# weiaicunzai/pytorch-camvid

Measured on AMD Instinct MI355X. Metric: images/sec fwd+bwd UNet 3x360x480 bs=8, higher is better.
Workload: dtype f32; 1 GPU; UNET(3,12) train fwd+bwd+CE, per-GPU batch 8 x 3x360x480 fp32 (BASELINE.json configs[1]); global_batch=8, parallelism=dp1

## Files before the change

pytorch-camvid_amd/csrc/pointwise.hip:

```cpp
#include "cvk_common.h"

namespace {

inline int grid_for(long total) {
    const long b = (total + 255) / 256;
    return (int)(b < 16384 ? (b > 0 ? b : 1) : 16384);
}

#define CVK_GRID_STRIDE(i, total) \
    for (long i = (long)blockIdx.x * blockDim.x + threadIdx.x; i < (total); i += (long)gridDim.x * blockDim.x)

__global__ void k_import_small(const float* __restrict__ src, int64_t sN, int64_t sC, int64_t sH, int64_t sW,
                               float* __restrict__ dst, int N, int C, int H, int W) {
    const long total = (long)N * H * W;
    CVK_GRID_STRIDE(i, total) {
        const int x = (int)(i % W);
        const long t = i / W;
        const int y = (int)(t % H), n = (int)(t / H);
        const float* p = src + n * sN + y * sH + x * sW;
        f32x4 v = {0.f, 0.f, 0.f, 0.f};
        for (int c = 0; c < C; ++c) v[c] = p[c * sC];
        *reinterpret_cast<f32x4*>(dst + i * 4) = v;
    }
}
// ... 279 lines not shown
        const int yo = (int)(t % Ho);
        t /= Ho;
        const int c = (int)(t % C), n = (int)(t / C);
        const int k = code[(((long)n * Ho + yo) * Wo + xo) * C + c];
        idx[i] = (int64_t)(2 * yo + (k >> 1)) * W + 2 * xo + (k & 1);
    }
}

struct Tap { int i0, i1; float l0, l1; };
__device__ __forceinline__ Tap make_tap(int dst, float scale, int n_in) {
    Tap t;
    const float src = scale * (float)dst;
    t.i0 = (int)src;
    if (t.i0 > n_in - 1) t.i0 = n_in - 1;
    t.i1 = t.i0 + (t.i0 < n_in - 1 ? 1 : 0);
    t.l1 = src - (float)t.i0;
    t.l0 = 1.f - t.l1;
    return t;
}

struct RowDiv {
    unsigned lo, hi_mask;
    explicit RowDiv(unsigned d) {
        const unsigned long long m = 0x100000000ULL / d + 1ULL;
        lo = (unsigned)m;
        hi_mask = (m >> 32) ? 0xFFFFFFFFu : 0u;
    }
    __device__ __forceinline__ unsigned div(unsigned t) const { return __umulhi(t, lo) + (t & hi_mask); }
};

template <int V>
__global__ __launch_bounds__(256) void k_bilinear_fwd(const float* __restrict__ x, float* __restrict__ out, int H, int W, int C,
                                                     float sy, float sx, RowDiv dcv) {
    typedef typename VT_<V>::T VT;
    const int Wo = 2 * W, cvn = C / V;
    const int yo = blockIdx.y, n = blockIdx.z;
    const unsigned idx = blockIdx.x * 256 + threadIdx.x;
    if (idx >= (unsigned)(Wo * cvn)) return;
    const int xo = (int)dcv.div(idx), cv = (int)idx - xo * cvn;
    const Tap ty = make_tap(yo, sy, H), tx = make_tap(xo, sx, W);
    const float* b = x + ((long)n * H * W) * C + cv * V;
    VT v00 = *reinterpret_cast<const VT*>(b + ((long)ty.i0 * W + tx.i0) * C);
    VT v01 = *reinterpret_cast<const VT*>(b + ((long)ty.i0 * W + tx.i1) * C);
    VT v10 = *reinterpret_cast<const VT*>(b + ((long)ty.i1 * W + tx.i0) * C);
    VT v11 = *reinterpret_cast<const VT*>(b + ((long)ty.i1 * W + tx.i1) * C);
    VT o;
#pragma unroll
    for (int j = 0; j < V; ++j)
        el<V>(o, j) = ty.l0 * (tx.l0 * el<V>(v00, j) + tx.l1 * el<V>(v01, j)) +
                      ty.l1 * (tx.l0 * el<V>(v10, j) + tx.l1 * el<V>(v11, j));
    *reinterpret_cast<VT*>(out + (((long)n * 2 * H + yo) * Wo) * C + (long)idx * V) = o;
}

constexpr int BL_TY = 4, BL_TX = 32, BL_IY = 4, BL_IX = 18;
__global__ __launch_bounds__(256) void k_bilinear_fwd_tiled(const float* __restrict__ x, float* __restrict__ out, int H, int W, int C,
                                                           float sy, float sx, int tilesX) {
    __shared__ f32x4 tile[BL_IY * BL_IX * 16];
    const int Ho = 2 * H, Wo = 2 * W;
    const int tx = blockIdx.x % tilesX, ty = blockIdx.x / tilesX, c0 = blockIdx.y * 64, n = blockIdx.z;
    const int yo0 = ty * BL_TY, xo0 = tx * BL_TX;
    const int iy0 = make_tap(yo0, sy, H).i0, ix0 = make_tap(xo0, sx, W).i0;
    const int t = threadIdx.x, cv = t & 15;
    const float* const xb = x + ((long)n * H * W) * C + c0 + cv * 4;
    for (int p = t >> 4; p < BL_IY * BL_IX; p += 16) {
        const int ry = p / BL_IX, rx = p - ry * BL_IX;
        const int iy = min(iy0 + ry, H - 1), ix = min(ix0 + rx, W - 1);
        tile[p * 16 + cv] = *reinterpret_cast<const f32x4*>(xb + ((long)iy * W + ix) * C);
    }
    __syncthreads();
    for (int p = t >> 4; p < BL_TY * BL_TX; p += 16) {
        const int oy = p / BL_TX, ox = p - oy * BL_TX;
        const int yo = yo0 + oy, xo = xo0 + ox;
        if (yo >= Ho || xo >= Wo) continue;
        const Tap ty_ = make_tap(yo, sy, H), tx_ = make_tap(xo, sx, W);
        const int r0 = (ty_.i0 - iy0) * BL_IX, r1 = (ty_.i1 - iy0) * BL_IX, q0 = tx_.i0 - ix0, q1 = tx_.i1 - ix0;
        const f32x4 v00 = tile[(r0 + q0) * 16 + cv], v01 = tile[(r0 + q1) * 16 + cv];
        const f32x4 v10 = tile[(r1 + q0) * 16 + cv], v11 = tile[(r1 + q1) * 16 + cv];
        f32x4 o;
#pragma unroll
        for (int j = 0; j < 4; ++j) o[j] = ty_.l0 * (tx_.l0 * v00[j] + tx_.l1 * v01[j]) + ty_.l1 * (tx_.l0 * v10[j] + tx_.l1 * v11[j]);
        *reinterpret_cast<f32x4*>(out + (((long)n * Ho + yo) * Wo + xo) * C + c0 + cv * 4) = o;
    }
}

template <int V>
__global__ __launch_bounds__(256) void k_bilinear_bwd(const float* __restrict__ dout, float* __restrict__ dx, int H, int W, int C,
                                                     float sy, float sx, RowDiv dcv, int gx, RowDiv dgx) {
    typedef typename VT_<V>::T VT;
    const int Ho = 2 * H, Wo = 2 * W, cvn = C / V;
    const unsigned lid = (unsigned)cvk_xcd_remap(blockIdx.x, gridDim.x);
    const unsigned row = dgx.div(lid), bx = lid - row * gx;
    const int n = (int)(row / (unsigned)H), yi = (int)(row - (unsigned)n * H);
    const unsigned idx = bx * 256 + threadIdx.x;
    if (idx >= (unsigned)(W * cvn)) return;
    const int xi = (int)dcv.div(idx), cv = (int)idx - xi * cvn;
    float wy[6], wx[6];
#pragma unroll
    for (int k = 0; k < 6; ++k) {
        const int yo = 2 * yi - 2 + k, xo = 2 * xi - 2 + k;
        wy[k] = 0.f; wx[k] = 0.f;
        if ((unsigned)yo < (unsigned)Ho) {
            const Tap t = make_tap(yo, sy, H);
            wy[k] = (t.i0 == yi ? t.l0 : 0.f) + (t.i1 == yi ? t.l1 : 0.f);
        }
        if ((unsigned)xo < (unsigned)Wo) {
            const Tap t = make_tap(xo, sx, W);
            wx[k] = (t.i0 == xi ? t.l0 : 0.f) + (t.i1 == xi ? t.l1 : 0.f);
// ... 250 lines not shown
```

pytorch-camvid_amd/csrc/wino2d.hip:

```cpp
#include "cvk_common.h"
#include "lds_dma.h"
#include "split_fmt.h"

namespace {

constexpr int W2_BN = 128;
__host__ __device__ inline int w2_tb(int T) { return T >= 8192 ? 16 : 4; }

template <typename T>
__host__ __device__ __forceinline__ void w2_bt(const T* d, T* v) {
    const T a = d[4] - 4.f * d[2], b = d[3] - 4.f * d[1], c = d[4] - d[2], e = 2.f * (d[3] - d[1]);
    v[0] = 4.f * d[0] - 5.f * d[2] + d[4];
    v[1] = a + b;
    v[2] = a - b;
    v[3] = c + e;
    v[4] = c - e;
    v[5] = 4.f * d[1] - 5.f * d[3] + d[5];
}
template <typename T>
__device__ __forceinline__ void w2_at(const T* m, T* y) {
    const T s12 = m[1] + m[2], d12 = m[1] - m[2], s34 = m[3] + m[4], d34 = m[3] - m[4];
    y[0] = m[0] + s12 + s34;
    y[1] = d12 + 2.f * d34;
    y[2] = s12 + 4.f * s34;
// ... 22 lines not shown
}

template <typename T>
__host__ __device__ __forceinline__ void w6_bt(const T* d, T* v) {
    v[0] = d[0] - d[6] + 5.25f * (d[4] - d[2]);
    v[7] = d[7] - d[1] + 5.25f * (d[3] - d[5]);
    const T a1 = d[2] + d[6] - 4.25f * d[4], b1 = d[1] + d[5] - 4.25f * d[3];
    v[1] = a1 + b1;
    v[2] = a1 - b1;
    const T a2 = d[6] + 0.25f * d[2] - 1.25f * d[4], b2 = 0.5f * d[1] - 2.5f * d[3] + 2.f * d[5];
    v[3] = a2 + b2;
    v[4] = a2 - b2;
    const T a3 = d[6] + 4.f * d[2] - 5.f * d[4], b3 = 2.f * d[1] - 2.5f * d[3] + 0.5f * d[5];
    v[5] = a3 + b3;
    v[6] = a3 - b3;
}
template <typename T>
__device__ __forceinline__ void w6_at(const T* m, T* y) {
    const T s12 = m[1] + m[2], d12 = m[1] - m[2], s34 = m[3] + m[4], d34 = m[3] - m[4], s56 = m[5] + m[6], d56 = m[5] - m[6];
    y[0] = m[0] + s12 + s34 + s56;
    y[1] = d12 + 2.f * d34 + 0.5f * d56;
    y[2] = s12 + 4.f * s34 + 0.25f * s56;
    y[3] = d12 + 8.f * d34 + 0.125f * d56;
    y[4] = s12 + 16.f * s34 + 0.0625f * s56;
    y[5] = d12 + 32.f * d34 + 0.03125f * d56 + m[7];
}
__host__ __device__ __forceinline__ void w6_g(const float* g, float* u) {
    const float t = g[0] + g[2];
    u[0] = g[0];
    u[1] = (-2.f / 9.f) * (t + g[1]);
    u[2] = (-2.f / 9.f) * (t - g[1]);
    const float q = (1.f / 90.f) * g[0] + (2.f / 45.f) * g[2];
    u[3] = q + (1.f / 45.f) * g[1];
    u[4] = q - (1.f / 45.f) * g[1];
    const float r = (32.f / 45.f) * g[0] + (8.f / 45.f) * g[2];
    u[5] = r + (16.f / 45.f) * g[1];
    u[6] = r - (16.f / 45.f) * g[1];
    u[7] = g[2];
}
template <typename T>
__host__ __device__ __forceinline__ void w6_a(const T* d, T* e) {
    const T ev = d[0] + d[2] + d[4], od = d[1] + d[3] + d[5];
    e[0] = d[0];
    e[1] = ev + od;
    e[2] = ev - od;
    const T ev2 = d[0] + 4.f * d[2] + 16.f * d[4], od2 = 2.f * d[1] + 8.f * d[3] + 32.f * d[5];
    e[3] = ev2 + od2;
    e[4] = ev2 - od2;
    const T ev3 = d[0] + 0.25f * d[2] + 0.0625f * d[4], od3 = 0.5f * d[1] + 0.125f * d[3] + 0.03125f * d[5];
    e[5] = ev3 + od3;
    e[6] = ev3 - od3;
    e[7] = d[5];
}
__device__ __forceinline__ void w6_gt(const float* p, float* w) {
    const float s12 = p[1] + p[2], d12 = p[1] - p[2], s34 = p[3] + p[4], d34 = p[3] - p[4], s56 = p[5] + p[6], d56 = p[5] - p[6];
    w[0] = p[0] - (2.f / 9.f) * s12 + (1.f / 90.f) * s34 + (32.f / 45.f) * s56;
    w[1] = -(2.f / 9.f) * d12 + (1.f / 45.f) * d34 + (16.f / 45.f) * d56;
    w[2] = -(2.f / 9.f) * s12 + (2.f / 45.f) * s34 + (8.f / 45.f) * s56 + p[7];
}
__device__ __forceinline__ void w2_gt(const float* m, float* w) {
    const float s12 = m[1] + m[2], d12 = m[2] - m[1], s34 = m[3] + m[4], d34 = m[3] - m[4];
    w[0] = 0.25f * m[0] - (1.f / 6.f) * s12 + (1.f / 24.f) * s34;
    w[1] = (1.f / 6.f) * d12 + (1.f / 12.f) * d34;
    w[2] = -(1.f / 6.f) * s12 + (1.f / 6.f) * s34 + m[5];
}

typedef float f32x2v __attribute__((ext_vector_type(2)));

template <int MT> struct W2T;
template <> struct W2T<4> {
    static constexpr int NT = 6, NX = 36, VW = 4;
    typedef f32x4 VT;
    template <typename T> static __host__ __device__ __forceinline__ void bt(const T* d, T* v) { w2_bt(d, v); }
    template <typename T> static __host__ __device__ __forceinline__ void a(const T* d, T* e) { w2_a(d, e); }
    static __host__ __device__ __forceinline__ void g(const float* x, float* u) { w2_g(x, u); }
    static __device__ __forceinline__ void gt(const float* x, float* w) { w2_gt(x, w); }
    static __device__ __forceinline__ constexpr float at(int r, int c) {
        return c == 0 ? (r == 0 ? 1.f : 0.f) : c == 5 ? (r == 3 ? 1.f : 0.f)
             : c == 1 ? 1.f : c == 2 ? ((r & 1) ? -1.f : 1.f)
             : c == 3 ? (float)(1 << r) : ((r & 1) ? -(float)(1 << r) : (float)(1 << r));
    }
};
template <> struct W2T<6> {
    static constexpr int NT = 8, NX = 64, VW = 2;
    typedef f32x2v VT;
    template <typename T> static __host__ __device__ __forceinline__ void bt(const T* d, T* v) { w6_bt(d, v); }
    template <typename T> static __host__ __device__ __forceinline__ void a(const T* d, T* e) { w6_a(d, e); }
    static __host__ __device__ __forceinline__ void g(const float* x, float* u) { w6_g(x, u); }
    static __device__ __forceinline__ void gt(const float* x, float* w) { w6_gt(x, w); }
    static __device__ __forceinline__ constexpr float at(int r, int c) {
        return c == 0 ? (r == 0 ? 1.f : 0.f) : c == 7 ? (r == 5 ? 1.f : 0.f)
             : c == 1 ? 1.f : c == 2 ? ((r & 1) ? -1.f : 1.f)
             : c == 3 ? (float)(1 << r) : c == 4 ? ((r & 1) ? -(float)(1 << r) : (float)(1 << r))
             : c == 5 ? 1.f / (float)(1 << r) : ((r & 1) ? -1.f / (float)(1 << r) : 1.f / (float)(1 << r));
    }
};

struct SplitDst {
    unsigned short* base;
    size_t term, xstride;
    unsigned amax;
    CvkSplitTab tab;
};
template <int VW, int FMT>
__device__ __forceinline__ SplitDst split_dst(void* S, int C, int Rpad, int t, int c, const unsigned* amax, const CvkSplitTab& tab) {
    const int ncs = C >> 5, cs = c >> 5, cl = c & 31;
    const int pos = (cl >> 3) ^ (((t >> 2) & 1) << 1);
    SplitDst d;
    d.term = (size_t)Rpad * 32;
    d.xstride = (size_t)ncs * FMT * d.term;
    d.base = reinterpret_cast<unsigned short*>(S) + ((size_t)cs * FMT * Rpad + t) * 32 + pos * 8 + (cl & 7);
    d.amax = FMT == 2 ? cvk_amax_read(amax) : 0u;
    d.tab = tab;
    return d;
}
__device__ __forceinline__ unsigned short w2_bf16_rne(float v) {
    const unsigned u = __builtin_bit_cast(unsigned, v);
    return (unsigned short)((u + 0x7FFFu + ((u >> 16) & 1u)) >> 16);
}
template <int FMT>
__device__ __forceinline__ unsigned short split_term(float& r) {
    if (FMT == 2) {
        const _Float16 h = (_Float16)r;
        r -= (float)h;
        return __builtin_bit_cast(unsigned short, h);
    }
    const unsigned short b = w2_bf16_rne(r);
    r -= __builtin_bit_cast(float, (unsigned)b << 16);
    return b;
}
template <int VW, int FMT, typename VT>
__device__ __forceinline__ void split_store(const SplitDst& d, int xi, int i, int j, VT v) {
    float r[VW];
    const float sc = FMT == 2 ? cvk_pow2f(cvk_split_exp(d.amax, cvk_split_tab_c(d.tab, i), cvk_split_tab_c(d.tab, j))) : 1.f;
#pragma unroll
    for (int q = 0; q < VW; ++q) r[q] = FMT == 2 ? v[q] * sc : v[q];
    unsigned short* p = d.base + (size_t)xi * d.xstride;
#pragma unroll
    for (int k = 0; k < FMT; ++k) {
        unsigned short b[VW];
#pragma unroll
        for (int q = 0; q < VW; ++q) b[q] = split_term<FMT>(r[q]);
// ... 501 lines not shown
    for (int i = 0; i < 2; ++i)
#pragma unroll
        for (int j = 0; j < 2; ++j)
#pragma unroll
            for (int e = 0; e < 16; ++e) acc[i][j][e] = 0.f;
    const int a_off = h * 512 + (wm * 64 + 2 * r) * 4, b_off = 16384 + h * 512 + (wn * 64 + 2 * r) * 4;
    typedef float f32x2 __attribute__((ext_vector_type(2)));

    if (kb < ke) issue(kb, 0);
    int buf = 0;
    for (int ks = kb; ks < ke; ++ks) {
        if (ABL != 2) cvk_wait_vm<0>();
        if (ABL != 1) cvk_lds_retire_barrier();
        const int ksn = ABL == 5 ? kb : min(ks + 1, ke - 1);
        if (!CVK_TN_SPLIT_ISSUE && ABL != 2) issue(ksn, buf ^ 1);
        __builtin_amdgcn_s_setprio(1);
        const char* const st = smem + buf * STAGE;
#pragma unroll
        for (int q = 0; q < 16; ++q) {
            f32x2 a, b;
            if (ABL == 4) { a = f32x2{acc[0][0][0], 1.f}; b = f32x2{acc[0][0][1], 2.f}; asm volatile("" : "+v"(a), "+v"(b)); }
            else {
                a = *reinterpret_cast<const f32x2*>(st + a_off + q * 1024);
                b = *reinterpret_cast<const f32x2*>(st + b_off + q * 1024);
            }
            if (CVK_TN_SPLIT_ISSUE && ABL != 2 && (q == 0 || q == 4)) {
#pragma unroll
                for (int p = (q ? PPW / 2 : 0); p < (q ? PPW : PPW / 2); ++p)
                    cvk_dma16(src[p] + (size_t)ksn * sstep[p], smem_addr + (buf ^ 1) * STAGE + (wave * PPW + p) * 1024);
            }
#pragma unroll
            for (int i = 0; i < 2; ++i)
#pragma unroll
                for (int j = 0; j < 2; ++j) acc[i][j] = __builtin_amdgcn_mfma_f32_32x32x2f32(a[i], b[j], acc[i][j], 0, 0, 0);
        }
        __builtin_amdgcn_s_setprio(0);
        buf ^= 1;
    }
    cvk_wait_vm<0>();
    const int col = tn * 128 + wn * 64 + 2 * r;
#pragma unroll
    for (int i = 0; i < 2; ++i)
#pragma unroll
        for (int e = 0; e < 16; ++e) {
            const int row = tm * 128 + wm * 64 + 2 * ((e & 3) + 8 * (e >> 2) + 4 * h) + i;
            if (ABL == 3 ? (row < Mm && acc[i][0][e] == 123.456f) : row < Mm) {
                float* const dp = D + (size_t)row * Nn + col;
                if (col + 1 < Nn) { const f32x2 v = {acc[i][0][e], acc[i][1][e]}; *reinterpret_cast<f32x2*>(dp) = v; }
                else if (col < Nn) dp[0] = acc[i][0][e];
            }
        }
}

template <int MT>
__global__ __launch_bounds__(256) void k_w2d_wgrad_out(const float* __restrict__ P, float* __restrict__ dw, int Co, int Ci, int Cip, int f) {
    typedef W2T<MT> TR;
    constexpr int NT = TR::NT, NX = TR::NX;
    const size_t total = (size_t)Co * Ci, plane = (size_t)Co * Cip;
    for (size_t idx = (size_t)blockIdx.x * 256 + threadIdx.x; idx < total; idx += (size_t)gridDim.x * 256) {
        const int ci = (int)(idx % Ci);
        const size_t co = idx / Ci;
        const float* const pp = P + co * Cip + ci;
        float mx[NX];
#pragma unroll
        for (int q = 0; q < NX; ++q) mx[q] = pp[(size_t)q * plane];
        for (int k = 1; k < f; ++k) {
            float v[NX];
#pragma unroll
            for (int q = 0; q < NX; ++q) v[q] = pp[(size_t)(k * NX + q) * plane];
#pragma unroll
            for (int q = 0; q < NX; ++q) mx[q] += v[q];
        }
        float t[NT][3];
#pragma unroll
        for (int a = 0; a < NT; ++a) TR::gt(mx + a * NT, t[a]);
#pragma unroll
        for (int kx = 0; kx < 3; ++kx) {
            float col[NT], w3[3];
#pragma unroll
            for (int a = 0; a < NT; ++a) col[a] = t[a][kx];
            TR::gt(col, w3);
            dw[(co * 9 + 0 + kx) * Ci + ci] = w3[0];
            dw[(co * 9 + 3 + kx) * Ci + ci] = w3[1];
            dw[(co * 9 + 6 + kx) * Ci + ci] = w3[2];
        }
    }
}

template <int MT, bool STATS>
__global__ __launch_bounds__(256) void k_w2d_output(const float* __restrict__ Mo, int ldm, const float* __restrict__ bias,
                                                   float* __restrict__ Y, int ldy, float* __restrict__ stats,
                                                   float* __restrict__ counts, int P, int H, int W, int th, int tw, int T,
                                                   int Cout, int cvn, int BM, int tmn, int tilesN, int split_start, int f) {
    typedef W2T<MT> TR;
    typedef typename TR::VT VT;
    constexpr int NT = TR::NT, NX = TR::NX, VW = TR::VW;
    __shared__ float red[2][256 * VW];
    const int t = threadIdx.x;
    const int pl = 256 / cvn, cv = t % cvn, lanep = t / cvn;
    const int c = (blockIdx.y * cvn + cv) * VW;
    const bool cok = c < Cout;
    VT sh = {};
    if (cok && bias != nullptr) sh = *reinterpret_cast<const VT*>(bias + c);
    VT s1 = {}, s2 = {};
    const size_t plane = (size_t)T * ldm;
    const int TB = w2_tb(T);
    const int tile_end = min(T, (int)(blockIdx.x + 1) * TB);
    for (int tile = blockIdx.x * TB + lanep; tile < tile_end && cok; tile += pl) {
        const int n = tile / (th * tw), rr = tile - n * th * tw, ty = rr / tw, tx = rr - ty * tw;
        const float* const mp = Mo + (size_t)tile * ldm + c;
        const int xi0 = f > 1 ? (split_start - ((tile / BM) * tilesN + c / W2_BN) + tmn - 1) / tmn : NX;
        VT o[MT][MT];
#pragma unroll
        for (int i = 0; i < MT; ++i)
#pragma unroll
            for (int jj = 0; jj < MT; ++jj) o[i][jj] = VT{};
#pragma unroll
        for (int j = 0; j < NT; ++j) {
            VT m[NT], z[MT];
#pragma unroll
            for (int i = 0; i < NT; ++i) {
                m[i] = *reinterpret_cast<const VT*>(mp + (size_t)(i * NT + j) * plane);
                if (i * NT + j >= xi0)
                    for (int k = 1; k < f; ++k) m[i] += *reinterpret_cast<const VT*>(mp + (size_t)(k * NX + i * NT + j) * plane);
            }
            if constexpr (MT == 4) {
                w2_at(m, z);
#pragma unroll
                for (int i = 0; i < 4; ++i) {
                    if (j == 0) { o[i][0] = z[i]; }
                    else if (j == 1) { o[i][0] += z[i]; o[i][1] = z[i]; o[i][2] = z[i]; o[i][3] = z[i]; }
                    else if (j == 2) { o[i][0] += z[i]; o[i][1] -= z[i]; o[i][2] += z[i]; o[i][3] -= z[i]; }
                    else if (j == 3) { o[i][0] += z[i]; o[i][1] += 2.f * z[i]; o[i][2] += 4.f * z[i]; o[i][3] += 8.f * z[i]; }
                    else if (j == 4) { o[i][0] += z[i]; o[i][1] -= 2.f * z[i]; o[i][2] += 4.f * z[i]; o[i][3] -= 8.f * z[i]; }
                    else { o[i][3] += z[i]; }
                }
            } else {
                w6_at(m, z);
#pragma unroll
// ... 202 lines not shown
    W2WPlan p;
    p.Tpad = w2_tpad(T);
    p.tilesM = cvk_cdiv(Cout, 128);
    p.tilesN = cvk_cdiv(Cin_pad, 128);
    const int nt = nx * p.tilesM * p.tilesN, nK = p.Tpad / 32;
    int f = cvk_cdiv(1024, nt);
    if (f > nK / 4) f = nK / 4;
    if (f > 16) f = 16;
    if (f < 1) f = 1;
    p.f = f;
    return p;
}

static int w2i_wgrad_ksplit(int mt, int T, int Cin_pad, int Cout) {
    if (T <= 0 || Cin_pad <= 0 || Cout <= 0) return 0;
    return plan_w2d_wgrad(w2_nx(mt), T, Cin_pad, Cout).f;
}

static int w2i_dy_transform(int mt, const char* who, const float* dy, int ld_dy, float* E, int N, int H, int W, int Cout, void* stream) {
    CVK_CHECK_ARG(dy && E && N > 0 && H > 0 && W > 0 && Cout >= 4 && Cout % 4 == 0 && ld_dy >= Cout && ld_dy % 4 == 0, "%s: bad arguments", who);
    CVK_CHECK_ARG(cvk_aligned16(dy) && cvk_aligned16(E), "%s: pointers must be 16-byte aligned", who);
    const int th = (H + mt - 1) / mt, tw = (W + mt - 1) / mt, T = N * th * tw, Tpad = w2_tpad(T);
    const long threads = (long)Tpad * (Cout / (mt == 4 ? 4 : 2));
    const dim3 grid((unsigned)((threads + 255) / 256));
    if (mt == 4) hipLaunchKernelGGL(k_w2d_dy<4>, grid, dim3(256), 0, (hipStream_t)stream, dy, ld_dy, E, H, W, Cout, th, tw, T, Tpad);
    else hipLaunchKernelGGL(k_w2d_dy<6>, grid, dim3(256), 0, (hipStream_t)stream, dy, ld_dy, E, H, W, Cout, th, tw, T, Tpad);
    CVK_LAUNCH_RETURN(who);
}

static int w2i_gemm_tn(int mt, const char* who, const float* E, const float* V, float* P, int T, int Cin_pad, int Cout, void* stream) {
    CVK_CHECK_ARG(E && V && P && T > 0 && Cin_pad > 0 && Cin_pad % 4 == 0 && Cout > 0 && Cout % 4 == 0, "%s: bad arguments", who);
    CVK_CHECK_ARG(cvk_aligned16(E) && cvk_aligned16(V) && cvk_aligned16(P), "%s: pointers must be 16-byte aligned", who);
    const int nx = w2_nx(mt);
    const W2WPlan p = plan_w2d_wgrad(nx, T, Cin_pad, Cout);
#ifdef CVK_EXPERIMENTS
#define CVK_TN_ABL_GO(A_) hipLaunchKernelGGL(k_w2d_gemm_tn<A_>, dim3(nx * p.tilesM * p.tilesN * p.f), dim3(256), 0, (hipStream_t)stream, E, Cout, V, Cin_pad, P, p.Tpad, Cout, Cin_pad, p.tilesM, p.tilesN, p.f, nx)
    switch (cvk_knob("CVK_W2D_TN_ABL", 0)) {
        case 1: CVK_TN_ABL_GO(1); CVK_LAUNCH_RETURN(who);
        case 2: CVK_TN_ABL_GO(2); CVK_LAUNCH_RETURN(who);
        case 3: CVK_TN_ABL_GO(3); CVK_LAUNCH_RETURN(who);
        case 4: CVK_TN_ABL_GO(4); CVK_LAUNCH_RETURN(who);
        case 5: CVK_TN_ABL_GO(5); CVK_LAUNCH_RETURN(who);
        default: break;
    }
#endif
    hipLaunchKernelGGL(k_w2d_gemm_tn<0>, dim3(nx * p.tilesM * p.tilesN * p.f), dim3(256), 0, (hipStream_t)stream, E, Cout, V, Cin_pad, P, p.Tpad,
                       Cout, Cin_pad, p.tilesM, p.tilesN, p.f, nx);
    CVK_LAUNCH_RETURN(who);
}

static int w2i_wgrad_output(int mt, const char* who, const float* P, float* dw, int T, int Cin, int Cin_pad, int Cout, void* stream) {
    CVK_CHECK_ARG(P && dw && T > 0 && Cin > 0 && Cin <= Cin_pad && Cout > 0, "%s: bad arguments", who);
    const W2WPlan p = plan_w2d_wgrad(w2_nx(mt), T, Cin_pad, Cout);
    const size_t total = (size_t)Cout * Cin;
    const int blocks = (int)((total + 255) / 256 < 16384 ? (total + 255) / 256 : 16384);
    if (mt == 4) hipLaunchKernelGGL(k_w2d_wgrad_out<4>, dim3(blocks), dim3(256), 0, (hipStream_t)stream, P, dw, Cout, Cin, Cin_pad, p.f);
    else hipLaunchKernelGGL(k_w2d_wgrad_out<6>, dim3(blocks), dim3(256), 0, (hipStream_t)stream, P, dw, Cout, Cin, Cin_pad, p.f);
    CVK_LAUNCH_RETURN(who);
}

static size_t w2i_wgrad_workspace_bytes(int mt, int N, int H, int W, int Cin_pad, int Cout) {
    if (N <= 0 || H <= 0 || W <= 0 || Cin_pad <= 0 || Cout <= 0) return 0;
    const int nx = w2_nx(mt);
    const W2WPlan p = plan_w2d_wgrad(nx, w2_tiles(mt, N, H, W), Cin_pad, Cout);
    return ((size_t)nx * p.Tpad * ((size_t)Cin_pad + Cout) + 2 * 128 + (size_t)p.f * nx * Cout * Cin_pad) * sizeof(float);
}

static int w2i_dy_both(int mt, const char* who, const float* dy, int ld_dy, float* Vp, float* E, int N, int H, int W, int C, void* stream) {
    CVK_CHECK_ARG(dy && Vp && E && N > 0 && H > 0 && W > 0 && C >= 4 && C % 4 == 0 && ld_dy >= C && ld_dy % 4 == 0, "%s: bad arguments", who);
    CVK_CHECK_ARG(cvk_aligned16(dy) && cvk_aligned16(Vp) && cvk_aligned16(E), "%s: pointers must be 16-byte aligned", who);
    const int th = (H + mt - 1) / mt, tw = (W + mt - 1) / mt, T = N * th * tw, Tpad = w2_tpad(T);
    const long threads = (long)Tpad * (C / (mt == 4 ? 4 : 2));
    const dim3 grid((unsigned)((threads + 255) / 256));
    if (mt == 4) hipLaunchKernelGGL(k_w2d_dy_both<4>, grid, dim3(256), 0, (hipStream_t)stream, dy, ld_dy, Vp, E, H, W, C, th, tw, T, Tpad, Tpad, (const unsigned*)nullptr, CvkSplitTab{}, CvkSplitTab{});
    else hipLaunchKernelGGL(k_w2d_dy_both<6>, grid, dim3(256), 0, (hipStream_t)stream, dy, ld_dy, Vp, E, H, W, C, th, tw, T, Tpad, Tpad, (const unsigned*)nullptr, CvkSplitTab{}, CvkSplitTab{});
    CVK_LAUNCH_RETURN(who);
}

template <int MT>
static CvkSplitTab w2_split_tab(int kind) {
    typedef W2T<MT> TR;
    constexpr int NT = TR::NT;
    const int nin = kind == CVK_SPLIT_KIND_B ? NT : (kind == CVK_SPLIT_KIND_G ? 3 : MT);
    double rs[8] = {};
    for (int k = 0; k < nin; ++k) {
        float d[8] = {}, v[8] = {};
        d[k] = 1.f;
        if (kind == CVK_SPLIT_KIND_B) TR::bt(d, v);
        else if (kind == CVK_SPLIT_KIND_G) TR::g(d, v);
        else TR::a(d, v);
        for (int i = 0; i < NT; ++i) rs[i] += v[i] < 0.f ? -(double)v[i] : (double)v[i];
    }
    CvkSplitTab t;
    t.c8 = 0ull;
    t.nt = NT;
    for (int i = 0; i < NT; ++i) {
        int c = -20;
        while (rs[i] > ldexp(1.0, c) * (1.0 + 1e-6)) ++c;
        t.c8 |= (unsigned long long)(unsigned)(c + 64) << (8 * i);
    }
    return t;
}
CvkSplitTab cvk_split_tab(int tile, int kind) { return tile == 4 ? w2_split_tab<4>(kind) : w2_split_tab<6>(kind); }

extern "C" int cvk_split_scale_exponent(int tile, int kind, int xi, unsigned amax_bits) {
    if (!(tile == 4 || tile == 6) || kind < 0 || kind > 2 || xi < 0 || xi >= w2_nx(tile)) return 0;
    const CvkSplitTab t = cvk_split_tab(tile, kind);
    return cvk_split_exp(amax_bits, cvk_split_tab_c(t, xi / t.nt), cvk_split_tab_c(t, xi % t.nt));
}

// ... 115 lines not shown
    hipStream_t s = (hipStream_t)stream;
    const int Rp = cvk_split3_rows_pad(rows, 128);
    if (Rp != rows) {
        const hipError_t e = hipMemsetAsync(U, 0, (size_t)w2_nx(tile) * (cols / 32) * fmt * Rp * 64, s);
        if (e != hipSuccess) { cvk_set_error("%s: memset failed: %s", who, hipGetErrorString(e)); return (int)e; }
    }
    const CvkSplitTab tab = cvk_split_tab(tile, CVK_SPLIT_KIND_G);
    const unsigned* am = (const unsigned*)amax;
    if (dgrad) {
        const dim3 grid(cvk_cdiv(Cin, 32), cvk_cdiv(Cout, 32));
#define CVK_W2_WDS(MT_, F_) hipLaunchKernelGGL((k_w2d_weight_dgrad<MT_, F_>), grid, dim3(256), 0, s, w, (float*)U, Cout, Cin, am, tab)
        if (tile == 4) { if (fmt == 3) CVK_W2_WDS(4, 3); else CVK_W2_WDS(4, 2); }
        else           { if (fmt == 3) CVK_W2_WDS(6, 3); else CVK_W2_WDS(6, 2); }
#undef CVK_W2_WDS
    } else {
        const size_t total = (size_t)Cout * Cin;
        const int blocks = (int)((total + 255) / 256 < 16384 ? (total + 255) / 256 : 16384);
#define CVK_W2_WS(MT_, F_) hipLaunchKernelGGL((k_w2d_weight<MT_, F_>), dim3(blocks), dim3(256), 0, s, w, (float*)U, Cout, Cin, am, tab)
        if (tile == 4) { if (fmt == 3) CVK_W2_WS(4, 3); else CVK_W2_WS(4, 2); }
        else           { if (fmt == 3) CVK_W2_WS(6, 3); else CVK_W2_WS(6, 2); }
#undef CVK_W2_WS
    }
    CVK_LAUNCH_RETURN(who);
}
extern "C" int cvk_w2d_weight_transform_split3(int tile, const float* w, void* U3, float* tmp, int Cout, int Cin, int dgrad, void* stream) {
    (void)tmp;
    return cvk_w2d_weight_transform_split(3, tile, w, U3, nullptr, Cout, Cin, dgrad, stream);
}

extern "C" int cvk_w2d_output_plain(int tile, const float* Mo, const float* bias, float* y, float* stats, float* counts, int N, int H, int W,
                                    int Cout, int ldy, void* stream) {
    const char* who = "cvk_w2d_output_plain";
    CVK_CHECK_ARG((tile == 4 || tile == 6) && Mo && y && N > 0 && H > 0 && W > 0, "%s: bad arguments", who);
    CVK_CHECK_ARG(Cout >= 64 && Cout % 4 == 0 && ldy >= Cout && ldy % 4 == 0, "%s: needs Cout %% 4 == 0, Cout >= 64 (got %d)", who, Cout);
    CVK_CHECK_ARG((stats == nullptr) == (counts == nullptr), "%s: stats and counts go together", who);
    CVK_CHECK_ARG(cvk_aligned16(Mo) && cvk_aligned16(y), "%s: pointers must be 16-byte aligned", who);
    const int mt = tile, th = (H + mt - 1) / mt, tw = (W + mt - 1) / mt, T = N * th * tw;
    const int vw = mt == 4 ? 4 : 2, nv = Cout / vw;
    const int cvn = nv >= 64 ? 64 : (nv >= 32 ? 32 : 16);
    const int P = cvk_cdiv(T, w2_tb(T));
    const int tilesM = cvk_cdiv(T, 128), tilesN = cvk_cdiv(Cout, 128);
    dim3 grid(P, cvk_cdiv(nv, cvn));
    hipStream_t s = (hipStream_t)stream;
#define CVK_W2_OUTP(MT_, ST_) hipLaunchKernelGGL((k_w2d_output<MT_, ST_>), grid, dim3(256), 0, s, Mo, Cout, bias, y, ldy, stats, counts, P, H, W, th, tw, T, Cout, cvn, \
                                                 128, tilesM * tilesN, tilesN, tilesM * tilesN, 1)
    if (mt == 4) { if (stats) CVK_W2_OUTP(4, true); else CVK_W2_OUTP(4, false); }
    else         { if (stats) CVK_W2_OUTP(6, true); else CVK_W2_OUTP(6, false); }
#undef CVK_W2_OUTP
    CVK_LAUNCH_RETURN(who);
}

extern "C" int cvk_w2d_wgrad_output_f(int tile, const float* P, float* dw, int Cin, int Cin_pad, int Cout, int f, void* stream) {
    CVK_CHECK_ARG((tile == 4 || tile == 6) && P && dw && Cin > 0 && Cin <= Cin_pad && Cout > 0 && f >= 1 && f <= 64, "cvk_w2d_wgrad_output_f: bad arguments");
    const size_t total = (size_t)Cout * Cin;
    const int blocks = (int)((total + 255) / 256 < 16384 ? (total + 255) / 256 : 16384);
    if (tile == 4) hipLaunchKernelGGL(k_w2d_wgrad_out<4>, dim3(blocks), dim3(256), 0, (hipStream_t)stream, P, dw, Cout, Cin, Cin_pad, f);
    else hipLaunchKernelGGL(k_w2d_wgrad_out<6>, dim3(blocks), dim3(256), 0, (hipStream_t)stream, P, dw, Cout, Cin, Cin_pad, f);
    CVK_LAUNCH_RETURN("cvk_w2d_wgrad_output_f");
}

extern "C" int cvk_w2d_tiles(int N, int H, int W) { return w2i_tiles(4, N, H, W); }
extern "C" int cvk_w2d_stat_partials(int N, int H, int W) { return w2i_stat_partials(4, N, H, W); }
extern "C" int cvk_w2d_ksplit(int T, int Cin, int Cout) { return w2i_ksplit(4, T, Cin, Cout); }
extern "C" size_t cvk_conv3x3_w2d_workspace_bytes(int N, int H, int W, int Cin, int Cout) { return w2i_workspace_bytes(4, N, H, W, Cin, Cout); }
extern "C" int cvk_w2d_weight_transform(const float* w, float* U, int Cout, int Cin, void* stream) {
    return w2i_weight_transform(4, "cvk_w2d_weight_transform", w, U, Cout, Cin, stream);
}
extern "C" int cvk_w2d_weight_transform_dgrad(const float* w, float* U, int Cout, int Cin, void* stream) {
    return w2i_weight_transform_dgrad(4, "cvk_w2d_weight_transform_dgrad", w, U, Cout, Cin, stream);
}
extern "C" int cvk_w2d_input_transform(const float* x, float* V, int N, int H, int W, int Cin, void* stream) {
    return w2i_input_transform(4, "cvk_w2d_input_transform", x, V, N, H, W, Cin, stream);
}
extern "C" int cvk_w2d_gemm(const float* V, const float* U, float* Mo, int T, int Cin, int Cout, void* stream) {
    return w2i_gemm(4, "cvk_w2d_gemm", V, U, Mo, T, Cin, Cout, stream);
}
extern "C" int cvk_w2d_output(const float* Mo, const float* bias, float* y, float* stats, float* counts, int N, int H, int W,
                              int Cin, int Cout, int ldy, void* stream) {
    return w2i_output(4, "cvk_w2d_output", Mo, bias, y, stats, counts, N, H, W, Cin, Cout, ldy, stream);
}

extern "C" int cvk_conv3x3_w2d(const float* x, const float* U, const float* bias, float* y, float* stats, float* counts,
                               int N, int H, int W, int Cin, int Cout, int ldy, void* workspace, size_t workspace_bytes,
                               void* stream) {
    CVK_CHECK_ARG(workspace && N > 0 && H > 0 && W > 0, "cvk_conv3x3_w2d: bad arguments");
    CVK_CHECK_ARG(cvk_aligned16(workspace) && workspace_bytes >= cvk_conv3x3_w2d_workspace_bytes(N, H, W, Cin, Cout),
                  "cvk_conv3x3_w2d: workspace too small or misaligned");
    const int T = w2_tiles(4, N, H, W);
    float* const V = (float*)workspace;
    float* const Mo = V + (size_t)36 * w2_tpad(T) * Cin + 128;
    int rc = cvk_w2d_input_transform(x, V, N, H, W, Cin, stream);
    if (rc == CVK_OK) rc = cvk_w2d_gemm(V, U, Mo, T, Cin, Cout, stream);
    if (rc == CVK_OK) rc = cvk_w2d_output(Mo, bias, y, stats, counts, N, H, W, Cin, Cout, ldy, stream);
    return rc;
}

extern "C" int cvk_w2d_wgrad_ksplit(int T, int Cin_pad, int Cout) { return w2i_wgrad_ksplit(4, T, Cin_pad, Cout); }
extern "C" int cvk_w2d_dy_transform(const float* dy, int ld_dy, float* E, int N, int H, int W, int Cout, void* stream) {
    return w2i_dy_transform(4, "cvk_w2d_dy_transform", dy, ld_dy, E, N, H, W, Cout, stream);
}
extern "C" int cvk_w2d_dy_transform_both(const float* dy, int ld_dy, float* Vp, float* E, int N, int H, int W, int Cout, void* stream) {
    return w2i_dy_both(4, "cvk_w2d_dy_transform_both", dy, ld_dy, Vp, E, N, H, W, Cout, stream);
}
extern "C" int cvk_w2d_gemm_tn(const float* E, const float* V, float* P, int T, int Cin_pad, int Cout, void* stream) {
    return w2i_gemm_tn(4, "cvk_w2d_gemm_tn", E, V, P, T, Cin_pad, Cout, stream);
}
extern "C" int cvk_w2d_wgrad_output(const float* P, float* dw, int T, int Cin, int Cin_pad, int Cout, void* stream) {
    return w2i_wgrad_output(4, "cvk_w2d_wgrad_output", P, dw, T, Cin, Cin_pad, Cout, stream);
}
extern "C" size_t cvk_conv3x3_wgrad_w2d_workspace_bytes(int N, int H, int W, int Cin_pad, int Cout) {
// ... 55 lines not shown
```

Before: 247.8 images/s.

## Parallelize Winograd wgrad output transform across tile rows and vectorize channels

Rewrites the Winograd weight-gradient output kernel so each block splits the NT transform rows across warps of 32 threads. Each thread sums its row's partial products over the f splits with unrolled, optionally float4-vectorized loads, and the column transform is finished through shared memory. Previously one thread loaded all NX values serially, which gave low memory parallelism and heavy register use. Separately, the bilinear upsample tile is enlarged to 8 output rows to get more reuse per shared-memory load.

```diff
diff --git a/pytorch-camvid_amd/csrc/pointwise.hip b/pytorch-camvid_amd/csrc/pointwise.hip
--- a/pytorch-camvid_amd/csrc/pointwise.hip
+++ b/pytorch-camvid_amd/csrc/pointwise.hip
@@ -355,7 +355,7 @@
     *reinterpret_cast<VT*>(out + (((long)n * 2 * H + yo) * Wo) * C + (long)idx * V) = o;
 }
 
-constexpr int BL_TY = 4, BL_TX = 32, BL_IY = 4, BL_IX = 18;
+constexpr int BL_TY = 8, BL_TX = 32, BL_IY = 6, BL_IX = 18;
 __global__ __launch_bounds__(256) void k_bilinear_fwd_tiled(const float* __restrict__ x, float* __restrict__ out, int H, int W, int C,
                                                            float sy, float sx, int tilesX) {
     __shared__ f32x4 tile[BL_IY * BL_IX * 16];
diff --git a/pytorch-camvid_amd/csrc/wino2d.hip b/pytorch-camvid_amd/csrc/wino2d.hip
--- a/pytorch-camvid_amd/csrc/wino2d.hip
+++ b/pytorch-camvid_amd/csrc/wino2d.hip
@@ -98,14 +98,16 @@
     e[6] = ev3 - od3;
     e[7] = d[5];
 }
-__device__ __forceinline__ void w6_gt(const float* p, float* w) {
-    const float s12 = p[1] + p[2], d12 = p[1] - p[2], s34 = p[3] + p[4], d34 = p[3] - p[4], s56 = p[5] + p[6], d56 = p[5] - p[6];
+template <typename T>
+__device__ __forceinline__ void w6_gt(const T* p, T* w) {
+    const T s12 = p[1] + p[2], d12 = p[1] - p[2], s34 = p[3] + p[4], d34 = p[3] - p[4], s56 = p[5] + p[6], d56 = p[5] - p[6];
     w[0] = p[0] - (2.f / 9.f) * s12 + (1.f / 90.f) * s34 + (32.f / 45.f) * s56;
     w[1] = -(2.f / 9.f) * d12 + (1.f / 45.f) * d34 + (16.f / 45.f) * d56;
     w[2] = -(2.f / 9.f) * s12 + (2.f / 45.f) * s34 + (8.f / 45.f) * s56 + p[7];
 }
-__device__ __forceinline__ void w2_gt(const float* m, float* w) {
-    const float s12 = m[1] + m[2], d12 = m[2] - m[1], s34 = m[3] + m[4], d34 = m[3] - m[4];
+template <typename T>
+__device__ __forceinline__ void w2_gt(const T* m, T* w) {
+    const T s12 = m[1] + m[2], d12 = m[2] - m[1], s34 = m[3] + m[4], d34 = m[3] - m[4];
     w[0] = 0.25f * m[0] - (1.f / 6.f) * s12 + (1.f / 24.f) * s34;
     w[1] = (1.f / 6.f) * d12 + (1.f / 12.f) * d34;
     w[2] = -(1.f / 6.f) * s12 + (1.f / 6.f) * s34 + m[5];
@@ -120,7 +122,7 @@
     template <typename T> static __host__ __device__ __forceinline__ void bt(const T* d, T* v) { w2_bt(d, v); }
     template <typename T> static __host__ __device__ __forceinline__ void a(const T* d, T* e) { w2_a(d, e); }
     static __host__ __device__ __forceinline__ void g(const float* x, float* u) { w2_g(x, u); }
-    static __device__ __forceinline__ void gt(const float* x, float* w) { w2_gt(x, w); }
+    template <typename T> static __device__ __forceinline__ void gt(const T* x, T* w) { w2_gt(x, w); }
     static __device__ __forceinline__ constexpr float at(int r, int c) {
         return c == 0 ? (r == 0 ? 1.f : 0.f) : c == 5 ? (r == 3 ? 1.f : 0.f)
              : c == 1 ? 1.f : c == 2 ? ((r & 1) ? -1.f : 1.f)
@@ -133,7 +135,7 @@
     template <typename T> static __host__ __device__ __forceinline__ void bt(const T* d, T* v) { w6_bt(d, v); }
     template <typename T> static __host__ __device__ __forceinline__ void a(const T* d, T* e) { w6_a(d, e); }
     static __host__ __device__ __forceinline__ void g(const float* x, float* u) { w6_g(x, u); }
-    static __device__ __forceinline__ void gt(const float* x, float* w) { w6_gt(x, w); }
+    template <typename T> static __device__ __forceinline__ void gt(const T* x, T* w) { w6_gt(x, w); }
     static __device__ __forceinline__ constexpr float at(int r, int c) {
         return c == 0 ? (r == 0 ? 1.f : 0.f) : c == 7 ? (r == 5 ? 1.f : 0.f)
              : c == 1 ? 1.f : c == 2 ? ((r & 1) ? -1.f : 1.f)
@@ -741,39 +743,68 @@
         }
 }
 
-template <int MT>
+template <int V> struct WgVec { typedef float T; };
+template <> struct WgVec<4> { typedef f32x4 T; };
+template <int MT, int V>
 __global__ __launch_bounds__(256) void k_w2d_wgrad_out(const float* __restrict__ P, float* __restrict__ dw, int Co, int Ci, int Cip, int f) {
     typedef W2T<MT> TR;
-    constexpr int NT = TR::NT, NX = TR::NX;
-    const size_t total = (size_t)Co * Ci, plane = (size_t)Co * Cip;
-    for (size_t idx = (size_t)blockIdx.x * 256 + threadIdx.x; idx < total; idx += (size_t)gridDim.x * 256) {
-        const int ci = (int)(idx % Ci);
-        const size_t co = idx / Ci;
-        const float* const pp = P + co * Cip + ci;
-        float mx[NX];
-#pragma unroll
-        for (int q = 0; q < NX; ++q) mx[q] = pp[(size_t)q * plane];
-        for (int k = 1; k < f; ++k) {
-            float v[NX];
-#pragma unroll
-            for (int q = 0; q < NX; ++q) v[q] = pp[(size_t)(k * NX + q) * plane];
-#pragma unroll
-            for (int q = 0; q < NX; ++q) mx[q] += v[q];
-        }
-        float t[NT][3];
-#pragma unroll
-        for (int a = 0; a < NT; ++a) TR::gt(mx + a * NT, t[a]);
-#pragma unroll
-        for (int kx = 0; kx < 3; ++kx) {
-            float col[NT], w3[3];
-#pragma unroll
-            for (int a = 0; a < NT; ++a) col[a] = t[a][kx];
-            TR::gt(col, w3);
-            dw[(co * 9 + 0 + kx) * Ci + ci] = w3[0];
-            dw[(co * 9 + 3 + kx) * Ci + ci] = w3[1];
-            dw[(co * 9 + 6 + kx) * Ci + ci] = w3[2];
-        }
-    }
+    typedef typename WgVec<V>::T VT;
+    constexpr int NT = TR::NT, NX = TR::NX, KU = 4;
+    __shared__ VT sh[NT][3][32];
+    const int lane = threadIdx.x & 31, a = threadIdx.x >> 5;
+    const int cvn = Ci / V;
+    const size_t nv = (size_t)Co * cvn, plane = (size_t)Co * Cip;
+    const size_t g = (size_t)blockIdx.x * 32 + lane;
+    const bool live = g < nv;
+    const size_t co = live ? g / cvn : 0;
+    const int ci = live ? (int)(g - co * cvn) * V : 0;
+    if (live) {
+        const float* const pp = P + co * Cip + ci + (size_t)(a * NT) * plane;
+        VT mx[NT] = {};
+        for (int k0 = 0; k0 < f; k0 += KU) {
+            VT v[KU][NT];
+#pragma unroll
+            for (int u = 0; u < KU; ++u) {
+                if (k0 + u < f) {
+#pragma unroll
+                    for (int b = 0; b < NT; ++b) v[u][b] = *reinterpret_cast<const VT*>(pp + ((size_t)(k0 + u) * NX + b) * plane);
+                }
+            }
+#pragma unroll
+            for (int u = 0; u < KU; ++u) {
+                if (k0 + u < f) {
+#pragma unroll
+                    for (int b = 0; b < NT; ++b) mx[b] = (k0 + u == 0) ? v[u][b] : mx[b] + v[u][b];
+                }
+            }
+        }
+        VT t[3];
+        TR::gt(mx, t);
+#pragma unroll
+        for (int kx = 0; kx < 3; ++kx) sh[a][kx][lane] = t[kx];
+    }
+    __syncthreads();
+    if (threadIdx.x < 96 && live) {
+        const int kx = a;
+        VT col[NT], w3[3];
+#pragma unroll
+        for (int r = 0; r < NT; ++r) col[r] = sh[r][kx][lane];
+        TR::gt(col, w3);
+#pragma unroll
+        for (int r = 0; r < 3; ++r) *reinterpret_cast<VT*>(dw + (co * 9 + 3 * r + kx) * Ci + ci) = w3[r];
+    }
+}
+
+static inline bool w2_wgrad_out_v4(const float* P, const float* dw, int Cin, int Cin_pad) {
+    return Cin % 4 == 0 && Cin_pad % 4 == 0 && cvk_aligned16(P) && cvk_aligned16(dw);
+}
+template <int MT>
+static void w2_launch_wgrad_out(const float* P, float* dw, int Cout, int Cin, int Cin_pad, int f, hipStream_t s) {
+    constexpr int NT = W2T<MT>::NT;
+    if (w2_wgrad_out_v4(P, dw, Cin, Cin_pad))
+        hipLaunchKernelGGL((k_w2d_wgrad_out<MT, 4>), dim3((unsigned)cvk_cdiv((long)Cout * (Cin / 4), 32)), dim3(32 * NT), 0, s, P, dw, Cout, Cin, Cin_pad, f);
+    else
+        hipLaunchKernelGGL((k_w2d_wgrad_out<MT, 1>), dim3((unsigned)cvk_cdiv((long)Cout * Cin, 32)), dim3(32 * NT), 0, s, P, dw, Cout, Cin, Cin_pad, f);
 }
 
 template <int MT, bool STATS>
@@ -1082,10 +1113,9 @@
 static int w2i_wgrad_output(int mt, const char* who, const float* P, float* dw, int T, int Cin, int Cin_pad, int Cout, void* stream) {
     CVK_CHECK_ARG(P && dw && T > 0 && Cin > 0 && Cin <= Cin_pad && Cout > 0, "%s: bad arguments", who);
     const W2WPlan p = plan_w2d_wgrad(w2_nx(mt), T, Cin_pad, Cout);
-    const size_t total = (size_t)Cout * Cin;
-    const int blocks = (int)((total + 255) / 256 < 16384 ? (total + 255) / 256 : 16384);
-    if (mt == 4) hipLaunchKernelGGL(k_w2d_wgrad_out<4>, dim3(blocks), dim3(256), 0, (hipStream_t)stream, P, dw, Cout, Cin, Cin_pad, p.f);
-    else hipLaunchKernelGGL(k_w2d_wgrad_out<6>, dim3(blocks), dim3(256), 0, (hipStream_t)stream, P, dw, Cout, Cin, Cin_pad, p.f);
+    CVK_CHECK_ARG((long)Cout * Cin < (1L << 31), "%s: too many filter elements for the grid", who);
+    if (mt == 4) w2_launch_wgrad_out<4>(P, dw, Cout, Cin, Cin_pad, p.f, (hipStream_t)stream);
+    else w2_launch_wgrad_out<6>(P, dw, Cout, Cin, Cin_pad, p.f, (hipStream_t)stream);
     CVK_LAUNCH_RETURN(who);
 }
 
@@ -1307,10 +1337,9 @@
 
 extern "C" int cvk_w2d_wgrad_output_f(int tile, const float* P, float* dw, int Cin, int Cin_pad, int Cout, int f, void* stream) {
     CVK_CHECK_ARG((tile == 4 || tile == 6) && P && dw && Cin > 0 && Cin <= Cin_pad && Cout > 0 && f >= 1 && f <= 64, "cvk_w2d_wgrad_output_f: bad arguments");
-    const size_t total = (size_t)Cout * Cin;
-    const int blocks = (int)((total + 255) / 256 < 16384 ? (total + 255) / 256 : 16384);
-    if (tile == 4) hipLaunchKernelGGL(k_w2d_wgrad_out<4>, dim3(blocks), dim3(256), 0, (hipStream_t)stream, P, dw, Cout, Cin, Cin_pad, f);
-    else hipLaunchKernelGGL(k_w2d_wgrad_out<6>, dim3(blocks), dim3(256), 0, (hipStream_t)stream, P, dw, Cout, Cin, Cin_pad, f);
+    CVK_CHECK_ARG((long)Cout * Cin < (1L << 31), "cvk_w2d_wgrad_output_f: too many filter elements for the grid");
+    if (tile == 4) w2_launch_wgrad_out<4>(P, dw, Cout, Cin, Cin_pad, f, (hipStream_t)stream);
+    else w2_launch_wgrad_out<6>(P, dw, Cout, Cin, Cin_pad, f, (hipStream_t)stream);
     CVK_LAUNCH_RETURN("cvk_w2d_wgrad_output_f");
 }
 
```

Result: no change. 247.8 images/s (median of 3 runs) (-0.0%).
